# HSU-ANT/gstpeaq

Measured on AMD Instinct MI355X. Metric: 2048-sample stereo ref/test frame-pairs/sec (basic PEAQ, ear model -> MOVs -> ODG); ODG delta vs CPU ref, higher is better.
Workload: dtype f64

## Files before the change

gstpeaq_amd/csrc/peaq_frontend.hip:

```cpp
#include <hip/hip_runtime.h>

#include "peaq_device.h"
#include "peaq_kernels.h"
#include <type_traits>

#include "peaq_wave.h"

namespace peaq {

#ifndef PEAQ_FE_PREFETCH_ITEMS
#define PEAQ_FE_PREFETCH_ITEMS 64
#endif
constexpr int kPrefetchItems = PEAQ_FE_PREFETCH_ITEMS;
constexpr int kUnitDoubles = 1288;
constexpr int kOffPw = 0;
constexpr int kOffScratch = 776;
constexpr int kPwLen = 776;
constexpr int kOffLogTab = 2 * kUnitDoubles;
constexpr int kLogTabDoubles = 2 * kLogTabEntries + 2;
constexpr int kLdsDoubles = 2 * kUnitDoubles + 2 * kLogTabDoubles;
#ifndef PEAQ_FE_WAVES
#define PEAQ_FE_WAVES 3
#endif
constexpr int kWavesPerSimd = PEAQ_FE_WAVES;

__device__ constexpr double kW32re[16] = {1., 0.98078528040323044913, 0.92387953251128675613, 0.83146961230254523708,
                                          0.70710678118654752440, 0.55557023301960222474, 0.38268343236508977173,
                                          0.19509032201612826785, 0., -0.19509032201612826785, -0.38268343236508977173,
                                          -0.55557023301960222474, -0.70710678118654752440, -0.83146961230254523708,
                                          -0.92387953251128675613, -0.98078528040323044913};
__device__ constexpr double kW32im[16] = {-0., -0.19509032201612826785, -0.38268343236508977173, -0.55557023301960222474,
                                          -0.70710678118654752440, -0.83146961230254523708, -0.92387953251128675613,
                                          -0.98078528040323044913, -1., -0.98078528040323044913, -0.92387953251128675613,
                                          -0.83146961230254523708, -0.70710678118654752440, -0.55557023301960222474,
                                          -0.38268343236508977173, -0.19509032201612826785};

__device__ __forceinline__ int pad16(int i) { return i + (i >> 4); }

__device__ __forceinline__ cplx tw_lane(const CommonTables* __restrict__ ct, int e, int lane) {
  const double2 v = *reinterpret_cast<const double2*>(ct->tw_lane[e][lane]);
  return {v.x, v.y};
}
__device__ __forceinline__ cplx csqr(cplx a) { return {a.re * a.re - a.im * a.im, 2. * (a.re * a.im)}; }

__device__ __forceinline__ void dft8_imag_upper(cplx (&x)[8]) {
  constexpr double c = 0.70710678118654752440;
  cplx a0 = {x[0].re, x[0].im + x[4].im}, a1 = {x[1].re, x[1].im + x[5].im};
  cplx a2 = {x[2].re, x[2].im + x[6].im}, a3 = {x[3].re, x[3].im + x[7].im};
  cplx b0 = {x[0].re, x[0].im - x[4].im}, b1 = {x[1].re, x[1].im - x[5].im};
  cplx b2 = {x[2].re, x[2].im - x[6].im}, b3 = {x[3].re, x[3].im - x[7].im};
  b1 = {c * (b1.re + b1.im), c * (b1.im - b1.re)};
  b2 = cmul_mi(b2);
  b3 = {c * (b3.im - b3.re), -c * (b3.re + b3.im)};
  dft4(a0, a1, a2, a3);
  dft4(b0, b1, b2, b3);
  x[0] = a0; x[2] = a1; x[4] = a2; x[6] = a3;
  x[1] = b0; x[3] = b1; x[5] = b2; x[7] = b3;
}

template <typename WR, typename RD>
__device__ __forceinline__ void exchange16(cplx (&z)[16], double* buf, WR wr, RD rd) {
#pragma unroll
  for (int r = 0; r < 16; ++r) buf[pad16(wr(r))] = z[r].re;
  wave_lds_fence();
#pragma unroll
  for (int r = 0; r < 16; ++r) z[r].re = buf[pad16(rd(r))];
  wave_lds_fence();
#pragma unroll
  for (int r = 0; r < 16; ++r) buf[pad16(wr(r))] = z[r].im;
  wave_lds_fence();
#pragma unroll
  for (int r = 0; r < 16; ++r) z[r].im = buf[pad16(rd(r))];
  wave_lds_fence();
}

template <typename F>
__device__ __forceinline__ void frame_power_spectrum(cplx (&z)[16], double (&p)[16], double* unit, int lane,
                                                     const CommonTables* __restrict__ ct,
                                                     double level_factor, F&& before_split) {
  const cplx w256 = tw_lane(ct, 2, lane);
  dft16(z);
  exchange16(z, unit, [&](int r) { return 16 * lane + r; }, [&](int r) { return lane + 64 * r; });
  {
    {
      cplx w[9];
      w[1] = w256;
      w[2] = csqr(w[1]);
      w[4] = csqr(w[2]);
      w[8] = csqr(w[4]);
      w[3] = cmul(w[1], w[2]);
      w[5] = cmul(w[4], w[1]);
      w[6] = cmul(w[4], w[2]);
      w[7] = cmul(w[4], w[3]);
#pragma unroll
      for (int r = 1; r < 8; ++r) {
        z[8 + r] = cmul(z[8 + r], cmul(w[8], w[r]));
        z[r] = cmul(z[r], w[r]);
      }
      z[8] = cmul(z[8], w[8]);
    }
    dft16(z);
#ifndef PEAQ_FE_LDS_EXCHANGE2
#pragma unroll
    for (int g = 0; g < 4; ++g) {
      rows_transpose4(z[4 * g].re, z[4 * g + 1].re, z[4 * g + 2].re, z[4 * g + 3].re);
      rows_transpose4(z[4 * g].im, z[4 * g + 1].im, z[4 * g + 2].im, z[4 * g + 3].im);
    }
#pragma unroll
    for (int a2 = 0; a2 < 4; ++a2)
#pragma unroll
      for (int g = a2 + 1; g < 4; ++g) {
        const cplx t = z[4 * a2 + g];
        z[4 * a2 + g] = z[4 * g + a2];
        z[4 * g + a2] = t;
      }
#else
    const int k = lane & 15, j = (lane - k) * 16 + k;
    exchange16(z, unit, [&](int r) { return j + 16 * r; },
               [&](int s) { return lane + 64 * (s & 3) + 256 * (s >> 2); });
#endif
  }
  const cplx wl = tw_lane(ct, 0, lane);
  double2 ew[8];
#pragma unroll
  for (int q = 0; q < 8; ++q) ew[q] = *reinterpret_cast<const double2*>(ct->ear_w2_pair[q][lane]);
  {
    constexpr double c1 = 0.92387953251128673848, s1 = 0.38268343236508977173, c2 = 0.70710678118654752440;
    const cplx wb = tw_lane(ct, 1, lane);
#pragma unroll
    for (int m = 0; m < 4; ++m) {
      const cplx w1 = m == 0 ? wb : m == 1 ? cmul(wb, {c1, -s1}) : m == 2 ? cmul(wb, {c2, -c2}) : cmul(wb, {s1, -c1});
      const cplx w2 = csqr(w1), w3 = cmul(w2, w1);
      z[m + 4] = cmul(z[m + 4], w1);
      z[m + 8] = cmul(z[m + 8], w2);
      z[m + 12] = cmul(z[m + 12], w3);
      dft4(z[m], z[m + 4], z[m + 8], z[m + 12]);
    }
  }
  before_split();
  wave_lds_fence();
  const int partner = (64 - lane) & 63;
  const double lf4 = 0.25 * level_factor;
#pragma unroll
  for (int q = 0; q < 8; ++q) {
    const int k = lane + 64 * q;
    cplx zm = {__shfl(z[15 - q].re, partner, 64), __shfl(z[15 - q].im, partner, 64)};
    if (lane == 0) zm = z[(16 - q) & 15];
    const cplx e2 = {z[q].re + zm.re, z[q].im - zm.im};
    const cplx o2 = {z[q].im + zm.im, zm.re - z[q].re};
    const cplx wq = {kW32re[q], kW32im[q]};
    const cplx t = cmul(q == 0 ? wl : cmul(wl, wq), o2);
    const cplx xp = cadd(e2, t), xm = csub(e2, t);
    p[q] = (xp.re * xp.re + xp.im * xp.im) * lf4;
    double pm = (xm.re * xm.re + xm.im * xm.im) * lf4;
    int km = 1024 - k;
    if (q == 0 && lane == 0) {
      pm = (z[8].re * z[8].re + z[8].im * z[8].im) * level_factor;
      km = 512;
    }
    p[8 + q] = pm;
    unit[kOffPw + k] = p[q] * ew[q].x;
    if (km < kPwLen) unit[kOffPw + km] = pm * ew[q].y;
  }
  wave_lds_fence();
}

__device__ __forceinline__ int spec_bin(int s, int lane) {
  if (s < 8) return lane + 64 * s;
  if (lane == 0 && s == 8) return 512;
  return 1024 - lane - 64 * (s - 8);
}

struct BandEdge {
  int lo, hi;
  double wlo, whi;
};
__device__ __forceinline__ BandEdge load_band_edge(const BandTables* __restrict__ bt, int b) {
  return {bt->lo[b], bt->hi[b], bt->wlo[b], bt->whi[b]};
}
__device__ __forceinline__ double group_band(const BandEdge& e, const double* sp, int zero) {
  const int lo = e.lo, hi = e.hi;
  double p = e.wlo * sp[lo] + e.whi * sp[hi];
  for (int k0 = lo + 1; k0 < hi; k0 += 8) {
    typedef const __attribute__((address_space(3))) double* lds_cptr;
    const lds_cptr q = (lds_cptr)sp + k0, z = (lds_cptr)sp + zero;
    const int n = hi - k0;
    double v[8];
#pragma unroll
    for (int j = 0; j < 8; ++j) {
      lds_cptr qj = j < n ? q : z - j;
      asm("" : "+v"(qj));
      v[j] = qj[j];
    }
#pragma unroll
    for (int j = 0; j < 8; ++j) p += v[j];
  }
// ... 192 lines not shown
  __builtin_amdgcn_s_setprio(0);
#ifdef PEAQ_FE_PROFILE
  asm volatile("s_waitcnt vmcnt(0)" ::: "memory");
#endif
  FE_MARK(14);
  wave_sum2(hop, energy, hop, energy);
  if (lane == 0) rec[sig ? kRecNoiseE : kRecSigE] = hop;
  const int energy_flag = energy >= 8000. / (32768. * 32768.);

  int above = 0;
  if (sig == 0) {
    if (__any((double)amax >= 200. / 32768 + 1e-6)) {
      above = 1;
    } else {
      float* ax = reinterpret_cast<float*>(unit);
      int lane_q = lane;
      asm volatile("" : "+v"(lane_q));
      const int voff_q = src.lane_offset(lane_q);
#pragma unroll
      for (int r = 0; r < 16; ++r) {
        const int n = lane_q + 64 * r;
        float x0, x1;
        src.load2(r, voff_q, x0, x1);
        reinterpret_cast<float2*>(ax)[n] = make_float2(fabsf(x0), fabsf(x1));
      }
      wave_lds_fence();
      above = boundary_detect(ax, kFrame, lane);
      wave_lds_fence();
    }
  }

  if (lane == 0)
    rec[sig ? kRecFlagsTest : kRecFlagsRef] = (double)(above | (energy_flag << 1));

  FE_MARK(0);
  double pspec[16];
  double2 lt0, lt1, lt2;
  frame_power_spectrum(z, pspec, unit, lane, ct, a.level_factor, [&] {
    lt0 = *reinterpret_cast<const double2*>(ct->log_tab[lane]);
    lt1 = *reinterpret_cast<const double2*>(ct->log_tab[64 + lane]);
    lt2 = *reinterpret_cast<const double2*>(ct->log_tab[128]);
  });
  const int gb1 = lane < (NB + 1) / 2 ? lane : 0, gb2 = lane < (NB + 1) / 2 ? NB - 1 - lane : 0;
  const BandEdge edge1 = load_band_edge(bt, gb1), edge2 = load_band_edge(bt, gb2);
  {
    reinterpret_cast<double2*>(ltab)[lane] = lt0;
    reinterpret_cast<double2*>(ltab)[64 + lane] = lt1;
    if (lane == 0) reinterpret_cast<double2*>(ltab)[128] = lt2;
    wave_lds_fence();
  }
  FE_MARK(1);
  constexpr bool kAdvanced = NB == 55;
  int bw_ref = 0, bw_test = 0;
  double* xch = lds + kOffLogTab + 2 * kLogTabEntries;
  double thr = 0.;
  auto top_bin = [&](double level, int limit, bool or_equal) {
    bool hit512 = false;
#pragma unroll
    for (int q = 0; q < 8; ++q) {
      unsigned long long m = __ballot(or_equal ? pspec[8 + q] >= level : pspec[8 + q] > level);
      if (q == 0) {
        hit512 = (m & 1ull) && 512 < limit;
        m &= ~1ull;
      }
      const int lo = 1024 - 64 * q - limit + 1;
      m &= lo >= 64 ? 0ull : lo <= 0 ? ~0ull : ~0ull << lo;
      if (m) return 1024 - 64 * q - __builtin_ctzll(m) + 1;
    }
    if (hit512) return 513;
#pragma unroll
    for (int q = 7; q >= 0; --q) {
      unsigned long long m = __ballot(or_equal ? pspec[q] >= level : pspec[q] > level);
      const int nl = limit - 64 * q;
      m &= nl >= 64 ? ~0ull : nl <= 0 ? 0ull : (1ull << nl) - 1ull;
      if (m) return 64 * q + 64 - __builtin_clzll(m);
    }
    return 0;
  };
  if (!kAdvanced && sig == 1) {
    if (lane >= 1) thr = pspec[8];
    if (lane <= 39) thr = fmax(thr, pspec[9]);
    thr = wave_max(thr);
    if (lane == 0) xch[0] = thr;
  }

  FE_MARK(2);
  const double* pw_ref = lds + kOffPw;
  double* pw_test = lds + kUnitDoubles + kOffPw;
  double* sa = lds + kOffScratch;
  double* sb = lds + kUnitDoubles + kOffScratch;
  int* adv_flag = reinterpret_cast<int*>(lds + kOffLogTab + kLogTabDoubles + 2 * kLogTabEntries);
  auto wait_flag = [&](int i) {
    while (__builtin_amdgcn_readfirstlane(*(volatile int*)(adv_flag + i)) == 0) __builtin_amdgcn_s_sleep(1);
    wave_lds_fence();
  };
  if constexpr (kAdvanced) {
    if (sig == 0 && lane == 0) {
      adv_flag[0] = 0;
      adv_flag[1] = 0;
    }
    __syncthreads();
    if (sig == 1) {
#pragma unroll
      for (int j = 0; j < 8; ++j) {
        const int k = lane + 64 * j;
        const double fr = pw_ref[k], ft = pw_test[k];
        sb[k] = (fr == 0. && ft == 0.) ? 0. : FE_LOG_NONNEG(ft / fr, ltab);
      }
      FE_MARK(8);
      wave_lds_fence();
      {
        constexpr int kSteps = (kPwLen + 63) / 64;
        double r[kSteps], t[kSteps];
#pragma unroll
        for (int i = 0; i < kSteps; ++i) {
          const int k = lane + 64 * i < kPwLen ? lane + 64 * i : 0;
          r[i] = pw_ref[k];
          t[i] = pw_test[k];
        }
        wave_lds_fence();
#pragma unroll
        for (int i = 0; i < kSteps; ++i)
          if (lane + 64 * i < kPwLen) pw_test[lane + 64 * i] = r[i] - 2 * sqrt_pos(r[i] * t[i]) + t[i];
      }
      wave_lds_fence();
      if (lane == 0) adv_flag[1] = 1;
      FE_MARK(10);
    }
  }
  if (!kAdvanced || sig == 0) {
    const double* pw = unit + kOffPw;
    constexpr int kZeroSlot = kOffScratch + 400 - kOffPw;
    if (lane == 0) scratch[400] = 0.;
    wave_lds_fence();
    double* ppx = scratch + 256;
    const int b0 = 2 * lane;
    double c_noise[2], c_lnauc[2], c_gil[2];
    const double c_dz02 = bt->dz02, c_ale = bt->aLe;
#pragma unroll
    for (int s2 = 0; s2 < 2; ++s2) {
      const int b = b0 + s2 < NB ? b0 + s2 : 0;
      c_noise[s2] = bt->internal_noise[b];
      c_lnauc[s2] = bt->ln_aUC[b];
      c_gil[s2] = bt->gIL[b];
    }
    if (lane < (NB + 1) / 2) {
      const int b1 = lane, b2 = NB - 1 - lane;
      ppx[b1] = group_band(edge1, pw, kZeroSlot);
      if (b2 != b1) ppx[b2] = group_band(edge2, pw, kZeroSlot);
    }
    wave_lds_fence();
    if (kAdvanced && lane == 0) adv_flag[0] = 1;
    FE_MARK(3);
    constexpr int kLanes = (NB - 1) / 2;
    double ene[2], ae[2], far[2], back2[2];
#pragma unroll
    for (int s = 0; s < 2; ++s) {
      const int b = b0 + s;
      if (b < NB) {
        const double pp = ppx[b] + c_noise[s];
        const double ln_pp = FE_LOG(pp, ltab);
        const double ln_a = c_lnauc[s] + c_dz02 * ln_pp;
        const double t = exp_fast(0.2 * ln_a), t2 = t * t;
        const double a_uce = t2 * t2 * t;
        const double g_iu = div_fast(1. - exp_fast((double)(NB - b) * ln_a), 1. - a_uce);
        ae[s] = t2;
        ene[s] = exp_fast(0.4 * (ln_pp - FE_LOG(c_gil[s] + g_iu - 1., ltab)));
        {
          double pw = 1., sq = t2;
#pragma unroll
          for (int e = 2 * kLanes - s; e; e >>= 1) {
            if (e & 1) pw *= sq;
            if (e >> 1) sq *= sq;
          }
          far[s] = ene[s] * pw;
        }
        const double t4 = t2 * t2;
        back2[s] = t4 > 1e-290 ? div_fast(1., t4) : 0.;
      } else {
        ae[s] = 0.;
        ene[s] = 0.;
        far[s] = 0.;
        back2[s] = 0.;
      }
    }
    FE_MARK(4);
    double up0 = 0., up1 = 0.;
    {
      double u = far[0], v = far[1];
#pragma unroll 9
      for (int k = kLanes; k >= 1; --k) {
        up0 += u;
        up0 += v;
        up1 = fma(ae[0], u, up1);
        up1 = fma(ae[1], v, up1);
        up0 = lane_below(up0);
        up1 = lane_below(up1);
        u *= back2[0];
        v *= back2[1];
      }
      up1 = fma(ae[0], ene[0], up1);
    }
    FE_MARK(5);
    double dn0, dn1;
    {
      const double al = c_ale;
      const double v = wave_suffix_geometric(ene[0] + al * ene[1], al * al, lane);
      const double nxt = lane_above(v);
      dn0 = v;
      dn1 = ene[1] + al * nxt;
    }
    double root[2];
#pragma unroll
    for (int s = 0; s < 2; ++s) {
      const double e2 = (s ? dn1 : dn0) + (s ? up1 : up0);
      root[s] = b0 + s < NB ? sqrt_pos(sqrt_pos(e2)) : 0.;
    }
    if (b0 < kBandStride)
      *reinterpret_cast<double2*>(rec + (sig ? kRecRootTest : kRecRootRef) + b0) = make_double2(root[0], root[1]);

  }
  FE_MARK(6);
  if constexpr (kAdvanced) {
    if (sig == 0) {
      const BandEdge e1 = load_band_edge(bt, gb1), e2 = load_band_edge(bt, gb2);
      if (lane == 0) xch[0] = 0.;
      wait_flag(1);
      const int zero_at = (int)(xch - pw_test);
      if (lane < (NB + 1) / 2) {
        const int b1 = lane, b2 = NB - 1 - lane;
        rec[kRecNoise + b1] = group_band(e1, pw_test, zero_at);
        if (b2 != b1) rec[kRecNoise + b2] = group_band(e2, pw_test, zero_at);
      } else if (lane < (NB + 1) / 2 + kBandStride - NB) {
        rec[kRecNoise + NB + lane - (NB + 1) / 2] = 0.;
      }
      if (lane == 0) {
        rec[kRecBwRef] = 0.;
        rec[kRecBwTest] = 0.;
      }
    } else {
      wait_flag(0);
    }
    FE_MARK(7);
  } else {
    __syncthreads();
    FE_MARK(7);
    if (sig == 0) {
      bw_ref = top_bin(10. * xch[0], 921, false);
      if (lane == 0) xch[1] = (double)bw_ref;
    }
  }

  if constexpr (!kAdvanced) {
    double* dlog = sa;
#ifndef PEAQ_FE_RATIOS_REF
#define PEAQ_FE_RATIOS_REF 3
#endif
    constexpr int kRefRatios = PEAQ_FE_RATIOS_REF;
    static_assert(kRefRatios >= 1 && kRefRatios <= 4, "the reference wave takes 1..4 of the 8 ratios per lane, the test wave the rest");
#pragma unroll
    for (int j = 0; j < 8 - kRefRatios; ++j) {
      if (sig == 0 && j >= kRefRatios) break;
      const int k = (sig == 0 ? 0 : 64 * kRefRatios) + lane + 64 * j;
      const double fr = pw_ref[k], ft = pw_test[k];
      dlog[k] = (fr == 0. && ft == 0.) ? 0. : FE_LOG_NONNEG(ft / fr, ltab);
    }
  }
  if constexpr (!kAdvanced) {
    FE_MARK(8);
    __syncthreads();
    FE_MARK(9);
  }
  if (!kAdvanced && sig == 1) {
    bw_ref = (int)xch[1];
    if (bw_ref > 346) bw_test = top_bin(3.16227766016838 * thr, bw_ref, true);
  }

  if (!kAdvanced && sig == 1) {
    wave_lds_fence();
    {
      constexpr int kSteps = (kPwLen + 63) / 64;
      double r[kSteps], t[kSteps];
#pragma unroll
      for (int i = 0; i < kSteps; ++i) {
        const int k = lane + 64 * i < kPwLen ? lane + 64 * i : 0;
        r[i] = pw_ref[k];
        t[i] = pw_test[k];
      }
      wave_lds_fence();
#pragma unroll
      for (int i = 0; i < kSteps; ++i)
        if (lane + 64 * i < kPwLen) pw_test[lane + 64 * i] = r[i] - 2 * sqrt_pos(r[i] * t[i]) + t[i];
      if (lane == 0) lds[kOffPw] = 0.;
    }
    wave_lds_fence();
    if (lane < (NB + 1) / 2) {
      const int b1 = lane, b2 = NB - 1 - lane;
      rec[kRecNoise + b1] = group_band(edge1, pw_test, kOffPw - kUnitDoubles);
      if (b2 != b1) rec[kRecNoise + b2] = group_band(edge2, pw_test, kOffPw - kUnitDoubles);
    } else if (lane < (NB + 1) / 2 + kBandStride - NB) {
      rec[kRecNoise + NB + lane - (NB + 1) / 2] = 0.;
    }
    if (lane == 0) {
      rec[kRecBwRef] = (double)bw_ref;
      rec[kRecBwTest] = (double)bw_test;
    }
    FE_MARK(10);
  } else if (kAdvanced ? sig == 1 : sig == 0) {
    double* const sa = kAdvanced ? lds + kOffPw : lds + kOffScratch;
    const cplx w64 = tw_lane(ct, 4, lane);
    const cplx w512 = tw_lane(ct, 3, lane);
    cplx ft1[3];
#pragma unroll
    for (int i = 0; i < 3; ++i) ft1[i] = tw_lane(ct, 5 + i, lane);
    cplx u[8];
    double g[4], run_in;
    {
      const double* d = kAdvanced ? sb : sa;
#pragma unroll
      for (int r = 0; r < 8; ++r) {
        const double v = d[lane + 64 * r];
        u[r] = {r < 4 ? v : 0., v};
      }
      double tot = 0.;
#pragma unroll
      for (int t = 0; t < 4; ++t) {
        const int j = 4 * lane + t;
        const double hi = d[j + 256], lo = d[j];
        g[t] = hi * hi - lo * lo;
        tot += g[t];
      }
      run_in = wave_prefix_sum(tot, lane) - tot;
    }
    wave_lds_fence();
    auto exchange8 = [&](auto wr, auto swz) {
#pragma unroll
      for (int r = 0; r < 8; ++r) {
        const int i = swz(wr(r));
        sa[i] = u[r].re;
        sb[i] = u[r].im;
      }
      wave_lds_fence();
#pragma unroll
      for (int r = 0; r < 8; ++r) {
        const int i = swz(lane + 64 * r);
        u[r] = {sa[i], sb[i]};
      }
      wave_lds_fence();
    };
    auto twiddle8 = [&](cplx w1) {
      cplx w[8];
      w[1] = w1;
// ... 167 lines not shown
```

gstpeaq_amd/csrc/peaq_wave.h:

```cpp
#pragma once
#include <hip/hip_runtime.h>

#include "peaq_device.h"

namespace peaq {

struct cplx {
  double re, im;
};

__device__ __forceinline__ cplx cadd(cplx a, cplx b) { return {a.re + b.re, a.im + b.im}; }
__device__ __forceinline__ cplx csub(cplx a, cplx b) { return {a.re - b.re, a.im - b.im}; }
__device__ __forceinline__ cplx cmul(cplx a, cplx b) {
  return {a.re * b.re - a.im * b.im, a.re * b.im + a.im * b.re};
}
__device__ __forceinline__ cplx cmul_mi(cplx a) { return {a.im, -a.re}; }

__device__ __forceinline__ void dft4(cplx& a0, cplx& a1, cplx& a2, cplx& a3) {
  const cplx t0 = cadd(a0, a2), t1 = csub(a0, a2), t2 = cadd(a1, a3), t3 = cmul_mi(csub(a1, a3));
  a0 = cadd(t0, t2);
  a1 = cadd(t1, t3);
  a2 = csub(t0, t2);
  a3 = csub(t1, t3);
}
// ... 64 lines not shown
  }
}
__device__ __forceinline__ void rows_transpose4_u(unsigned& x0, unsigned& x1, unsigned& x2, unsigned& x3) {
  auto r = __builtin_amdgcn_permlane32_swap(x0, x2, false, false);
  x0 = r[0];
  x2 = r[1];
  r = __builtin_amdgcn_permlane32_swap(x1, x3, false, false);
  x1 = r[0];
  x3 = r[1];
  r = __builtin_amdgcn_permlane16_swap(x0, x1, false, false);
  x0 = r[0];
  x1 = r[1];
  r = __builtin_amdgcn_permlane16_swap(x2, x3, false, false);
  x2 = r[0];
  x3 = r[1];
}
__device__ __forceinline__ void rows_transpose4(double& x0, double& x1, double& x2, double& x3) {
  unsigned l0 = __double2loint(x0), l1 = __double2loint(x1), l2 = __double2loint(x2), l3 = __double2loint(x3);
  unsigned h0 = __double2hiint(x0), h1 = __double2hiint(x1), h2 = __double2hiint(x2), h3 = __double2hiint(x3);
  rows_transpose4_u(l0, l1, l2, l3);
  rows_transpose4_u(h0, h1, h2, h3);
  x0 = __hiloint2double(h0, l0);
  x1 = __hiloint2double(h1, l1);
  x2 = __hiloint2double(h2, l2);
  x3 = __hiloint2double(h3, l3);
}

template <bool ROWS16>
__device__ __forceinline__ void swap_halves_d(double v, double& a, double& b) {
  int alo, blo, ahi, bhi;
  swap_halves_i<ROWS16>(__double2loint(v), alo, blo);
  swap_halves_i<ROWS16>(__double2hiint(v), ahi, bhi);
  a = __hiloint2double(ahi, alo);
  b = __hiloint2double(bhi, blo);
}
template <int CTRL>
__device__ __forceinline__ double dpp_d0(double v) {
  return __hiloint2double(__builtin_amdgcn_update_dpp(0, __double2hiint(v), CTRL, 0xF, 0xF, true),
                          __builtin_amdgcn_update_dpp(0, __double2loint(v), CTRL, 0xF, 0xF, true));
}
constexpr int kDppRowShl = 0x100, kDppRowShr = 0x110, kDppWaveShl1 = 0x130, kDppWaveShr1 = 0x138;
__device__ __forceinline__ double lane_below(double v) { return dpp_d0<kDppWaveShr1>(v); }
__device__ __forceinline__ double lane_above(double v) { return dpp_d0<kDppWaveShl1>(v); }
template <int L>
__device__ __forceinline__ double read_lane(double v) {
  return __hiloint2double(__builtin_amdgcn_readlane(__double2hiint(v), L), __builtin_amdgcn_readlane(__double2loint(v), L));
}
constexpr int kDppRowBcast15 = 0x142, kDppRowBcast31 = 0x143;
template <int CTRL, int ROWS>
__device__ __forceinline__ double dpp_rows_d0(double v) {
  return __hiloint2double(__builtin_amdgcn_update_dpp(0, __double2hiint(v), CTRL, ROWS, 0xF, false),
                          __builtin_amdgcn_update_dpp(0, __double2loint(v), CTRL, ROWS, 0xF, false));
}
template <int CTRL, int ROWS>
__device__ __forceinline__ double dpp_rows_keep(double v, double& z) {
  z = __hiloint2double(__builtin_amdgcn_update_dpp(__double2hiint(z), __double2hiint(v), CTRL, ROWS, 0xF, false),
                       __builtin_amdgcn_update_dpp(__double2loint(z), __double2loint(v), CTRL, ROWS, 0xF, false));
  return z;
}
__device__ __forceinline__ double row_carry_15(double v, double& z) { return dpp_rows_keep<kDppRowBcast15, 0xA>(v, z); }
__device__ __forceinline__ double row_carry_31(double v, double& z) { return dpp_rows_keep<kDppRowBcast31, 0xC>(v, z); }
__device__ __forceinline__ double row_carry_15(double v) { return dpp_rows_d0<kDppRowBcast15, 0xA>(v); }
__device__ __forceinline__ double row_carry_31(double v) { return dpp_rows_d0<kDppRowBcast31, 0xC>(v); }

__device__ __forceinline__ double wave_prefix_sum(double v, int lane) {
  v += dpp_d0<kDppRowShr + 1>(v);
  v += dpp_d0<kDppRowShr + 2>(v);
  v += dpp_d0<kDppRowShr + 4>(v);
  v += dpp_d0<kDppRowShr + 8>(v);
  v += row_carry_15(v);
  return v + row_carry_31(v);
}
__device__ __forceinline__ double wave_suffix_geometric(double v, double m, int lane) {
  double wl = 1., base = m;
  const int k = 16 - (lane & 15);
#pragma unroll
  for (int bit = 0; bit < 5; ++bit) {
    wl = (k >> bit) & 1 ? wl * base : wl;
    base *= base;
  }
  const double m16 = read_lane<0>(wl);
  v = fma(m, dpp_d0<kDppRowShl + 1>(v), v);
  m *= m;
  v = fma(m, dpp_d0<kDppRowShl + 2>(v), v);
  m *= m;
  v = fma(m, dpp_d0<kDppRowShl + 4>(v), v);
  m *= m;
  v = fma(m, dpp_d0<kDppRowShl + 8>(v), v);
  const double t3 = read_lane<48>(v);
  const double t2 = fma(m16, t3, read_lane<32>(v));
  const double t1 = fma(m16, t2, read_lane<16>(v));
  const int row = lane >> 4;
  return fma(wl, row == 0 ? t1 : row == 1 ? t2 : row == 2 ? t3 : 0., v);
}

__device__ __forceinline__ double wave_prefix_geometric(double v, double m1, double m2, double m4, double m8, double m16,
                                                        double wl, int lane) {
  v = fma(m1, dpp_d0<kDppRowShr + 1>(v), v);
  v = fma(m2, dpp_d0<kDppRowShr + 2>(v), v);
  v = fma(m4, dpp_d0<kDppRowShr + 4>(v), v);
  v = fma(m8, dpp_d0<kDppRowShr + 8>(v), v);
  v = fma(wl, row_carry_15(v), v);
  return fma((lane >> 4) == 3 ? wl * m16 : wl, row_carry_31(v), v);
}
__device__ __forceinline__ double wave_prefix_geometric(double v, double m1, double m2, double m4, double m8, double m16,
                                                        double wl, int lane, double& z15, double& z31) {
  v = fma(m1, dpp_d0<kDppRowShr + 1>(v), v);
  v = fma(m2, dpp_d0<kDppRowShr + 2>(v), v);
  v = fma(m4, dpp_d0<kDppRowShr + 4>(v), v);
  v = fma(m8, dpp_d0<kDppRowShr + 8>(v), v);
  v = fma(wl, row_carry_15(v, z15), v);
  return fma((lane >> 4) == 3 ? wl * m16 : wl, row_carry_31(v, z31), v);
}

template <int CTRL>
__device__ __forceinline__ float dpp_f0(float v) {
  return __int_as_float(__builtin_amdgcn_update_dpp(0, __float_as_int(v), CTRL, 0xF, 0xF, true));
}
__device__ __forceinline__ float wave_prefix_geometric(float v, float m1, float m2, float m4, float m8, float m16, float wl,
                                                       int lane) {
  v = fmaf(m1, dpp_f0<kDppRowShr + 1>(v), v);
  v = fmaf(m2, dpp_f0<kDppRowShr + 2>(v), v);
  v = fmaf(m4, dpp_f0<kDppRowShr + 4>(v), v);
  v = fmaf(m8, dpp_f0<kDppRowShr + 8>(v), v);
  const float t0 = __int_as_float(__builtin_amdgcn_readlane(__float_as_int(v), 15));
  const float t1 = fmaf(m16, t0, __int_as_float(__builtin_amdgcn_readlane(__float_as_int(v), 31)));
  const float t2 = fmaf(m16, t1, __int_as_float(__builtin_amdgcn_readlane(__float_as_int(v), 47)));
  const int row = lane >> 4;
  return fmaf(wl, row == 0 ? 0.f : row == 1 ? t0 : row == 2 ? t1 : t2, v);
}

template <typename OP>
__device__ __forceinline__ double wave_reduce_d(double v, OP op) {
  v = op(v, dpp_d<kDppXor1>(v));
  v = op(v, dpp_d<kDppXor2>(v));
  v = op(v, dpp_d<kDppHalfMirror>(v));
  v = op(v, dpp_d<kDppMirror>(v));
  double a, b;
  swap_halves_d<true>(v, a, b);
  v = op(a, b);
  swap_halves_d<false>(v, a, b);
  return op(a, b);
}
__device__ __forceinline__ double wave_sum(double v) {
  return wave_reduce_d(v, [](double x, double y) { return x + y; });
}
__device__ __forceinline__ double wave_max(double v) {
  return wave_reduce_d(v, [](double x, double y) { return fmax(x, y); });
}
__device__ __forceinline__ double fuse_halves_sum(double a, double b) {
  const auto lo = __builtin_amdgcn_permlane32_swap((unsigned)__double2loint(a), (unsigned)__double2loint(b), false, false);
  const auto hi = __builtin_amdgcn_permlane32_swap((unsigned)__double2hiint(a), (unsigned)__double2hiint(b), false, false);
  return __hiloint2double((int)hi[0], (int)lo[0]) + __hiloint2double((int)hi[1], (int)lo[1]);
}
__device__ __forceinline__ double fuse_rows_sum(double a, double b) {
  const auto lo = __builtin_amdgcn_permlane16_swap((unsigned)__double2loint(a), (unsigned)__double2loint(b), false, false);
  const auto hi = __builtin_amdgcn_permlane16_swap((unsigned)__double2hiint(a), (unsigned)__double2hiint(b), false, false);
  return __hiloint2double((int)hi[0], (int)lo[0]) + __hiloint2double((int)hi[1], (int)lo[1]);
}
__device__ __forceinline__ double row_sum_d(double v) {
  v += dpp_d<kDppXor1>(v);
  v += dpp_d<kDppXor2>(v);
  v += dpp_d<kDppHalfMirror>(v);
  v += dpp_d<kDppMirror>(v);
  return v;
}
__device__ __forceinline__ double lane_value_d(double v, int l) {
  return __hiloint2double(__builtin_amdgcn_readlane(__double2hiint(v), l), __builtin_amdgcn_readlane(__double2loint(v), l));
}
__device__ __forceinline__ void wave_sum2(double a, double b, double& sa, double& sb) {
  double v = fuse_halves_sum(a, b), p, q;
  swap_halves_d<true>(v, p, q);
  v = row_sum_d(p + q);
  sa = lane_value_d(v, 0);
  sb = lane_value_d(v, 32);
}
__device__ __forceinline__ void wave_sum4(double a, double b, double c, double d, double& sa, double& sb, double& sc,
                                          double& sd) {
  const double v = row_sum_d(fuse_rows_sum(fuse_halves_sum(a, b), fuse_halves_sum(c, d)));
  sa = lane_value_d(v, 0);
  sc = lane_value_d(v, 16);
  sb = lane_value_d(v, 32);
  sd = lane_value_d(v, 48);
}


#ifndef PEAQ_SK_DEFAULT
#define PEAQ_SK_DEFAULT false
#endif
template <long long BITS> __device__ __forceinline__ double scalar_const() {
  unsigned lo, hi;
  asm("s_mov_b32 %0, %1" : "=s"(lo) : "i"((unsigned)(BITS & 0xffffffffll)));
  asm("s_mov_b32 %0, %1" : "=s"(hi) : "i"((unsigned)((unsigned long long)BITS >> 32)));
  return __hiloint2double((int)hi, (int)lo);
}
#define PEAQ_KC(c) (SK ? scalar_const<__builtin_bit_cast(long long, (double)(c))>() : (double)(c))
__device__ __forceinline__ double fma_sgpr(double a, double b, double c_scalar) {
  double r;
  asm("v_fma_f64 %0, %1, %2, %3" : "=v"(r) : "v"(a), "v"(b), "s"(c_scalar));
  return r;
}
#define PEAQ_SC(c) scalar_const<__builtin_bit_cast(long long, (double)(c))>()
template <bool SK, long long BITS> __device__ __forceinline__ double fma_const(double a, double b) {
  if constexpr (SK) {
    double r;
    asm("v_fma_f64 %0, %1, %2, %3" : "=v"(r) : "v"(a), "v"(b), "s"(scalar_const<BITS>()));
    return r;
  } else {
    return fma(a, b, __builtin_bit_cast(double, BITS));
  }
}
#define PEAQ_FMA_KC(a, b, c) fma_const<SK, __builtin_bit_cast(long long, (double)(c))>(a, b)

template <bool SK = PEAQ_SK_DEFAULT> __device__ __forceinline__ double log_pos(double x) {
  double m = __builtin_amdgcn_frexp_mant(x);
  int e = __builtin_amdgcn_frexp_exp(x);
  const bool low = m < PEAQ_KC(0.70710678118654752440);
  m = low ? m + m : m;
  e = low ? e - 1 : e;
  const double num = m - 1., den = m + 1.;
  double r = __builtin_amdgcn_rcp(den);
  r = fma(fma(-den, r, 1.), r, r);
  double s = num * r;
  s = fma(fma(-den, s, num), r, s);
  const double z = s * s;
  double p = PEAQ_KC(1. / 19);
  p = PEAQ_FMA_KC(p, z, 1. / 17);
  p = PEAQ_FMA_KC(p, z, 1. / 15);
  p = PEAQ_FMA_KC(p, z, 1. / 13);
  p = PEAQ_FMA_KC(p, z, 1. / 11);
  p = PEAQ_FMA_KC(p, z, 1. / 9);
  p = PEAQ_FMA_KC(p, z, 1. / 7);
  p = PEAQ_FMA_KC(p, z, 1. / 5);
  p = PEAQ_FMA_KC(p, z, 1. / 3);
  const double t = s + s;
  const double lm = fma(t * z, p, t);
  const double ef = (double)e;
  return fma(ef, PEAQ_KC(6.93147180369123816490e-01), fma(ef, PEAQ_KC(1.90821492927058770002e-10), lm));
}

__device__ __forceinline__ double log_tab(double x, const double* __restrict__ tab) {
  const double m = __builtin_amdgcn_frexp_mant(x);
  int e = __builtin_amdgcn_frexp_exp(x);
  const unsigned idx = min(__builtin_amdgcn_ubfe((unsigned)__double2hiint(m) + 0x1000u, 13, 8), 128u);
  const double2 t = *reinterpret_cast<const double2*>(tab + 2 * idx);
  e -= idx < (unsigned)kLogTabFold ? 1 : 0;
  const double r = fma(m, t.x, -1.);
  constexpr bool SK = PEAQ_SK_DEFAULT;
  double p = -1. / 6;
  p = PEAQ_FMA_KC(p, r, 1. / 5);
  p = PEAQ_FMA_KC(p, r, -1. / 4);
  p = PEAQ_FMA_KC(p, r, 1. / 3);
  p = fma(p, r, -0.5);
  const double l1p = fma(r * r, p, r);
  return fma((double)e, PEAQ_KC(6.93147180559945286227e-01), t.y) + l1p;
}
#ifdef PEAQ_NO_LOGTAB_FE
#define FE_LOG(x, tab) log_pos(x)
#define FE_LOG_NONNEG(x, tab) log_nonneg(x)
#else
#define FE_LOG(x, tab) log_tab(x, tab)
#define FE_LOG_NONNEG(x, tab) log_tab_nonneg(x, tab)
#endif
__device__ __forceinline__ double log_tab_nonneg(double x, const double* __restrict__ tab) {
  const double l = log_tab(x, tab);
  return x == 0. ? -__builtin_inf() : (x == __builtin_inf() ? __builtin_inf() : l);
}

template <bool SK = PEAQ_SK_DEFAULT> __device__ __forceinline__ double log_nonneg(double x) {
  const double l = log_pos<SK>(x);
  return x == 0. ? -__builtin_inf() : (x == __builtin_inf() ? __builtin_inf() : l);
}

__device__ __forceinline__ double exp_tab(double x, const double* __restrict__ tab) {
  x = fmin(fmax(x, -1000.), 1000.);
  const double n = __builtin_rint(x * 9.23324826168936580e+01);
  double r = fma(-n, 6.93147180369123816490e-01 / 64, x);
  r = fma(-n, 1.90821492927058770002e-10 / 64, r);
  const int ni = (int)n;
  const double t = tab[ni & 63];
  double p = fma(r, 1. / 120., 1. / 24.);
  p = fma(p, r, 1. / 6.);
  p = fma(p, r, 0.5);
  p = fma(p, r, 1.);
  return __builtin_amdgcn_ldexp(fma(t, p * r, t), ni >> 6);
}
template <bool SK = PEAQ_SK_DEFAULT> __device__ __forceinline__ double exp_fast(double x) {
  x = fmin(fmax(x, -1000.), 1000.);
  const double n = __builtin_rint(x * PEAQ_KC(1.44269504088896338700e+00));
  double r = fma(-n, PEAQ_KC(6.93147180369123816490e-01), x);
  r = fma(-n, PEAQ_KC(1.90821492927058770002e-10), r);
  double p = PEAQ_KC(1. / 479001600.);
  p = PEAQ_FMA_KC(p, r, 1. / 39916800.);
  p = PEAQ_FMA_KC(p, r, 1. / 3628800.);
  p = PEAQ_FMA_KC(p, r, 1. / 362880.);
  p = PEAQ_FMA_KC(p, r, 1. / 40320.);
  p = PEAQ_FMA_KC(p, r, 1. / 5040.);
  p = PEAQ_FMA_KC(p, r, 1. / 720.);
  p = PEAQ_FMA_KC(p, r, 1. / 120.);
  p = PEAQ_FMA_KC(p, r, 1. / 24.);
  p = PEAQ_FMA_KC(p, r, 1. / 6.);
  p = fma(p, r, 0.5);
  p = fma(p, r, 1.);
  p = fma(p, r, 1.);
  return __builtin_amdgcn_ldexp(p, (int)n);
}
// ... 112 lines not shown
```

Baseline: 29.66 million.

## Split upward spreading chain across idle upper half-wave lanes

The serial upward-spreading recurrence, previously run over kLanes sequential lane-shift steps using only the lower lanes, is split in two. Idle lanes in the upper half of the wave take a copy of the far terms via permlane32 swap and process the longest-distance part of the chain in parallel. Their partial sums are then redistributed through LDS and added back after a shorter main loop. This shortens the dependent DPP shift chain, which is the latency bottleneck, at the cost of extra permlane swaps, an LDS round trip with a fence, and a more intricate schedule that is checked by constexpr static_asserts.

```diff
diff --git a/gstpeaq_amd/csrc/peaq_frontend.hip b/gstpeaq_amd/csrc/peaq_frontend.hip
--- a/gstpeaq_amd/csrc/peaq_frontend.hip
+++ b/gstpeaq_amd/csrc/peaq_frontend.hip
@@ -2,6 +2,7 @@
 
 #include "peaq_device.h"
 #include "peaq_kernels.h"
+#include "peaq_spread_sched.h"
 #include <type_traits>
 
 #include "peaq_wave.h"
@@ -42,6 +43,15 @@
   return {v.x, v.y};
 }
 __device__ __forceinline__ cplx csqr(cplx a) { return {a.re * a.re - a.im * a.im, 2. * (a.re * a.im)}; }
+__device__ __forceinline__ double pow_const(double x, int e) {
+  double pw = 1., sq = x;
+#pragma unroll
+  for (; e; e >>= 1) {
+    if (e & 1) pw *= sq;
+    if (e >> 1) sq *= sq;
+  }
+  return pw;
+}
 
 __device__ __forceinline__ void dft8_imag_upper(cplx (&x)[8]) {
   constexpr double c = 0.70710678118654752440;
@@ -540,8 +550,18 @@
     wave_lds_fence();
     if (kAdvanced && lane == 0) adv_flag[0] = 1;
     FE_MARK(3);
-    constexpr int kLanes = (NB - 1) / 2;
+    constexpr int kLanes = spread_lanes(NB);
+#ifdef PEAQ_FE_SPREAD_ONE_STREAM
+    constexpr int kHelper = 0, kFirst = kLanes, kBoundary = kLanes + 1;
+    constexpr int kExpUpper = 2 * kLanes, kExpHelper = 0;
+    constexpr int kUnrollMain = 9;
+#else
+    constexpr int kUnrollMain = 8;
+    constexpr int kHelper = spread_helper_steps(NB), kFirst = spread_k0(NB), kBoundary = spread_boundary(NB);
+    constexpr int kExpUpper = spread_exp_upper(NB, 0), kExpHelper = spread_exp_helper(NB);
+#endif
     double ene[2], ae[2], far[2], back2[2];
+    [[maybe_unused]] double far_copy[2], upper[2];
 #pragma unroll
     for (int s = 0; s < 2; ++s) {
       const int b = b0 + s;
@@ -554,14 +574,13 @@
         const double g_iu = div_fast(1. - exp_fast((double)(NB - b) * ln_a), 1. - a_uce);
         ae[s] = t2;
         ene[s] = exp_fast(0.4 * (ln_pp - FE_LOG(c_gil[s] + g_iu - 1., ltab)));
-        {
-          double pw = 1., sq = t2;
-#pragma unroll
-          for (int e = 2 * kLanes - s; e; e >>= 1) {
-            if (e & 1) pw *= sq;
-            if (e >> 1) sq *= sq;
-          }
-          far[s] = ene[s] * pw;
+        upper[s] = ene[s] * pow_const(t2, kExpUpper - s);
+        if constexpr (kHelper > 0) {
+          const double ph = pow_const(t2, kExpHelper);
+          far[s] = upper[s] * ph;
+          far_copy[s] = far[s] * ph;
+        } else {
+          far[s] = upper[s];
         }
         const double t4 = t2 * t2;
         back2[s] = t4 > 1e-290 ? div_fast(1., t4) : 0.;
@@ -569,6 +588,8 @@
         ae[s] = 0.;
         ene[s] = 0.;
         far[s] = 0.;
+        far_copy[s] = 0.;
+        upper[s] = 0.;
         back2[s] = 0.;
       }
     }
@@ -576,8 +597,39 @@
     double up0 = 0., up1 = 0.;
     {
       double u = far[0], v = far[1];
-#pragma unroll 9
-      for (int k = kLanes; k >= 1; --k) {
+      [[maybe_unused]] double2 home = make_double2(0., 0.);
+      if constexpr (kHelper > 0) {
+        u = lower_halves(far[0], far_copy[0]);
+        v = lower_halves(far[1], far_copy[1]);
+        const double wa0 = lower_halves(ae[0], ae[0]), wa1 = lower_halves(ae[1], ae[1]);
+        const double wb0 = lower_halves(back2[0], back2[0]), wb1 = lower_halves(back2[1], back2[1]);
+        const int act = lane < kSpreadHelperBase ? kLanes - lane : kFirst - (lane - kSpreadHelperBase);
+#pragma unroll 5
+        for (int k = kFirst; k >= kBoundary; --k) {
+          if (k <= act) {
+            asm volatile("");
+            up0 += u;
+            up0 += v;
+            up1 = fma(wa0, u, up1);
+            up1 = fma(wa1, v, up1);
+          }
+          up0 = lane_below(up0);
+          up1 = lane_below(up1);
+          u *= wb0;
+          v *= wb1;
+        }
+        const bool lower = lane < kSpreadHelperBase;
+        double2* hx = reinterpret_cast<double2*>(ppx);
+        hx[(lane + spread_home_shift(NB) + kSpreadWave) & (kSpreadWave - 1)] = lower ? make_double2(0., 0.) : make_double2(up0, up1);
+        wave_lds_fence();
+        home = hx[lane];
+        up0 = lower ? up0 : 0.;
+        up1 = lower ? up1 : 0.;
+        u = lower ? u : upper[0];
+        v = lower ? v : upper[1];
+      }
+#pragma unroll kUnrollMain
+      for (int k = kBoundary - 1; k >= 1; --k) {
         up0 += u;
         up0 += v;
         up1 = fma(ae[0], u, up1);
@@ -586,6 +638,10 @@
         up1 = lane_below(up1);
         u *= back2[0];
         v *= back2[1];
+      }
+      if constexpr (kHelper > 0) {
+        up0 += home.x;
+        up1 += home.y;
       }
       up1 = fma(ae[0], ene[0], up1);
     }
diff --git a/gstpeaq_amd/csrc/peaq_spread_sched.h b/gstpeaq_amd/csrc/peaq_spread_sched.h
--- /dev/null
+++ b/gstpeaq_amd/csrc/peaq_spread_sched.h
@@ -0,0 +1,46 @@
+#pragma once
+
+constexpr int kSpreadWave = 64;
+constexpr int kSpreadHelperBase = 32;
+
+constexpr int spread_lanes(int nb) { return (nb - 1) / 2; }
+constexpr int spread_helper_steps(int nb) {
+  const int by_half = (kSpreadHelperBase - 1) / 2, by_steps = spread_lanes(nb) / 2;
+  return by_half < by_steps ? by_half : by_steps;
+}
+constexpr int spread_k0(int nb) { return spread_lanes(nb) - spread_helper_steps(nb); }
+constexpr int spread_boundary(int nb) { return spread_k0(nb) - spread_helper_steps(nb) + 1; }
+constexpr int spread_act(int nb, int lane) {
+  return lane < kSpreadHelperBase ? spread_lanes(nb) - lane : spread_k0(nb) - (lane - kSpreadHelperBase);
+}
+constexpr int spread_home_shift(int nb) { return spread_helper_steps(nb) + spread_boundary(nb) - (kSpreadHelperBase + 1); }
+constexpr int spread_exp_upper(int nb, int s) { return 2 * (spread_boundary(nb) - 1) - s; }
+constexpr int spread_exp_helper(int nb) { return 2 * spread_helper_steps(nb); }
+constexpr int spread_exp_main(int nb, int s) { return spread_exp_upper(nb, s) + spread_exp_helper(nb); }
+
+constexpr bool spread_schedule_covers(int nb) {
+  const int kl = spread_lanes(nb), h = spread_helper_steps(nb), k0 = spread_k0(nb), kb = spread_boundary(nb);
+  if (h < 1 || kb < 2 || k0 + h != kl || kl >= kSpreadWave || kSpreadHelperBase + h > kSpreadWave) return false;
+  int count[kSpreadWave][kSpreadWave] = {};
+  for (int k = k0; k >= 1; --k) {
+    for (int lane = 0; lane < kSpreadWave; ++lane) {
+      const bool helper_phase = k >= kb;
+      if (helper_phase && k > spread_act(nb, lane)) continue;
+      const bool copy = helper_phase && lane >= kSpreadHelperBase;
+      const int src = copy ? lane - kSpreadHelperBase : lane, dist = copy ? k + h : k;
+      if (src + dist <= kl) {
+        ++count[src][dist];
+        if (helper_phase && !copy && lane + 1 >= kSpreadHelperBase) return false;
+      } else if (helper_phase) {
+        return false;
+      }
+      if (copy && lane + (k - kb + 1) + spread_home_shift(nb) != src + dist) return false;
+    }
+  }
+  for (int s = 0; s <= kl; ++s)
+    for (int k = 1; k < kSpreadWave; ++k)
+      if (count[s][k] != (s + k <= kl ? 1 : 0)) return false;
+  return spread_exp_main(nb, 0) == 2 * k0 && spread_exp_upper(nb, 1) >= 1;
+}
+static_assert(spread_schedule_covers(109) && spread_k0(109) == 39 && spread_boundary(109) == 25, "upward spreading, 109 bands");
+static_assert(spread_schedule_covers(55) && spread_k0(55) == 14 && spread_boundary(55) == 2, "upward spreading, 55 bands");
diff --git a/gstpeaq_amd/csrc/peaq_wave.h b/gstpeaq_amd/csrc/peaq_wave.h
--- a/gstpeaq_amd/csrc/peaq_wave.h
+++ b/gstpeaq_amd/csrc/peaq_wave.h
@@ -240,6 +240,11 @@
   const auto lo = __builtin_amdgcn_permlane32_swap((unsigned)__double2loint(a), (unsigned)__double2loint(b), false, false);
   const auto hi = __builtin_amdgcn_permlane32_swap((unsigned)__double2hiint(a), (unsigned)__double2hiint(b), false, false);
   return __hiloint2double((int)hi[0], (int)lo[0]) + __hiloint2double((int)hi[1], (int)lo[1]);
+}
+__device__ __forceinline__ double lower_halves(double a, double b) {
+  const auto lo = __builtin_amdgcn_permlane32_swap((unsigned)__double2loint(a), (unsigned)__double2loint(b), false, false);
+  const auto hi = __builtin_amdgcn_permlane32_swap((unsigned)__double2hiint(a), (unsigned)__double2hiint(b), false, false);
+  return __hiloint2double((int)hi[0], (int)lo[0]);
 }
 __device__ __forceinline__ double fuse_rows_sum(double a, double b) {
   const auto lo = __builtin_amdgcn_permlane16_swap((unsigned)__double2loint(a), (unsigned)__double2loint(b), false, false);
```

After: 30.38 million (median of 6 runs). 1.02x the previous value.
